# seervideodiffusion/SeerVideoLDM

Measured on AMD Instinct MI355X. Metric: UNet denoising steps/sec (12-frame 256^2 latent, 50-step DDIM), higher is better.
Workload: dtype bf16; 1 GPU; Sthv2 config: CFG batch 2 x 12 frames (2 cond + 10 predicted) x 32x32 latent, full-width SeerUNet 1.08G params, 50-step DDIM, scale 7.5; global_batch=1, parallelism=single, hip_graph=True

## Files before the change

### include/seer_hip.h

```cpp
#ifndef SEER_HIP_H
#define SEER_HIP_H

#include <stdint.h>

#ifdef __cplusplus
extern "C" {
#endif

#define SEER_OK 0
#define SEER_EINVAL (-22)
#define SEER_ENOSYS (-38)
#define SEER_ELAUNCH (-5)

#define SEER_DT_BF16 0
#define SEER_DT_F16 1

int seer_abi_version(void);
const char* seer_strerror(int code);
const char* seer_build_arch(void);

#define SEER_GEMM_PLAIN 0
#define SEER_GEMM_CONV3X3 1
#define SEER_EPI_GEGLU 1u
#define SEER_EPI_OUT_F32 2u
// ... 129 lines not shown

int64_t seer_groupnorm_workspace_floats(int32_t C, int32_t batch, int64_t rows_per_batch, int32_t groups);
int seer_groupnorm_stats(const void* x1, int32_t C1, const void* x2, int32_t C2, int32_t batch,
                         int64_t rows_per_batch, int32_t groups, float* stats, float* workspace, int32_t dtype, void* stream);
int seer_groupnorm_stats_from_colsums(const float* cs1, int32_t C1, int32_t phases1, int32_t tiles1, const float* cs2,
                                      int32_t C2, int32_t phases2, int32_t tiles2, int32_t batch, int32_t groups,
                                      float* stats, void* stream);
int seer_groupnorm_apply(const void* x1, int32_t C1, const void* x2, int32_t C2, int32_t batch,
                         int64_t rows_per_batch, int32_t groups, const float* stats, double count, float eps,
                         const float* gamma, const float* beta, int32_t silu, void* y, int32_t dtype, void* stream);
int seer_groupnorm_apply_from_colsums(const void* x1, int32_t C1, const void* x2, int32_t C2, const float* cs1, int32_t phases1,
                                      int32_t tiles1, const float* cs2, int32_t phases2, int32_t tiles2, int32_t batch,
                                      int64_t rows_per_batch, int32_t groups, double count, float eps, const float* gamma,
                                      const float* beta, int32_t silu, void* y, int32_t dtype, void* stream);
int seer_groupnorm_apply_fx(const void* x1, int32_t C1, const void* x2, int32_t C2, const int64_t* fx1, int32_t reps1,
                            const int64_t* fx2, int32_t reps2, int32_t batch, int64_t rows_per_batch, int32_t groups, double count, float eps, const float* gamma,
                            const float* beta, int32_t silu, void* y, float* stats_out, int32_t dtype, void* stream);
int seer_groupnorm_stats_fx(const void* x, int32_t C, int32_t batch, int64_t rows_per_batch, int64_t* fx, int32_t dtype,
                            void* stream);
int seer_ff_fused_c320(const void* a, int32_t lda, const void* wof, const float* bo, const void* h, int32_t ldh, const void* x,
                       int32_t ldx, void* y, int32_t ldy, int64_t M, const float* gamma, const float* beta, float eps,
                       const void* w1f, const float* b1, const void* wcf, const float* bcat, int64_t* colsum_fx, int64_t fx_rows,
                       int32_t fx_reps, float* colsum_tiles, int32_t dtype, void* stream);
typedef struct seer_rowchain_desc {
    const void* inp; int32_t ld_in;
    const float* gn_stats; const int64_t* gn_fx; int32_t gn_fx_reps;
    double gn_count; float gn_eps; const float* gn_gamma; const float* gn_beta; int64_t rows_per_batch; int32_t groups;
    const void* w1f; const float* b1; const void* res; int32_t ldr; void* h; int32_t ldh;
    const float* ln_gamma; const float* ln_beta; float ln_eps;
    const void* w2f; int32_t n2; void* out; int32_t ldo;
    float col_scale; int32_t scale_thirds;
    const float* rot_table; int32_t rot_tokens_per_batch, rot_pos_offset, rot_head_dim, rot_dim, rot_thirds;
    int64_t M;
    int32_t dtype;
} seer_rowchain_desc;
int seer_rowchain_c320(const seer_rowchain_desc* desc , void* stream);
int seer_rowchain_pack(const void* W, int32_t ld, int32_t n_mats, void* out, void* stream);
int seer_ff_fused_pack_w1(const void* w1, void* out, void* stream);
int seer_ff_fused_pack_wcat(const void* wcat, void* out, void* stream);
int seer_layernorm(const void* x, int64_t rows, int32_t C, int32_t ldx, const float* gamma, const float* beta,
                   float eps, void* y, int32_t ldy, int32_t dtype, void* stream);

int seer_softmax_rows(const void* x, int32_t x_is_f32, int64_t rows, int32_t n, int32_t ld, float scale, void* y,
                      int32_t ldy, int32_t dtype, void* stream);

int seer_timestep_embedding(const int64_t* t, int32_t B, int32_t dim, int32_t flip_sin_to_cos, float freq_shift,
                            float* out, void* stream);

int seer_linear_smallm(const float* x, int32_t B, int32_t K, const void* W, const float* bias, int32_t N,
                       int32_t silu_in, int32_t silu_out, float* y, int32_t dtype, void* stream);

int seer_conv_in(const float* x, int32_t B, int32_t Cin, int32_t F, int32_t H, int32_t W_, const float* Wt,
                 const float* bias, int32_t Cout, void* y, int32_t dtype, void* stream);
int seer_conv_out(const void* x, int32_t B, int32_t C0, int32_t F, int32_t H, int32_t W_, const float* Wt,
                  const float* bias, int32_t Cout, float* y, int32_t dtype, void* stream);

int seer_conv1x1_nchw_f32(const float* x, int32_t N, int32_t Cin, int32_t Cout, int32_t HW, const float* Wt,
                          const float* bias, float* y, void* stream);

int seer_cast_f32(const float* x, int64_t n, void* y, int32_t dtype, void* stream);
int seer_nchw_f32_to_nhwc_bf16(const float* x, int32_t N, int32_t C, int32_t HW, void* y, void* stream);
int seer_nhwc_bf16_to_nchw_f32(const void* x, int32_t N, int32_t C, int32_t HW, float* y, void* stream);

int seer_cfg_ddim_step(const float* eps, int32_t cfg, int32_t b, int32_t C, int32_t F_total, int32_t cond_f,
                       int32_t HW, float scale, const float* coef, int32_t index, const float* x,
                       const float* noise , float* x_prev, float* pred_x0, void* stream);

int seer_ddim_step_begin(const float* x0_emb , const float* x, int32_t b, int32_t reps, int32_t C,
                         int32_t f1, int32_t F_pred, int32_t HW, const int64_t* t_table, int32_t* step, float* sample,
                         int64_t* t_out, void* stream);
int seer_cfg_ddim_step_dev(const float* eps, int32_t cfg, int32_t b, int32_t C, int32_t F_total, int32_t cond_f, int32_t HW,
                           float scale, const float* coef, int32_t* step, const float* x, const float* noise, float* x_prev,
                           float* pred_x0, void* stream);

int seer_slot_step_begin(const float* x0_emb , const float* x, int32_t slots, int32_t reps, int32_t C,
                         int32_t f1, int32_t F_pred, int32_t HW, const int64_t* t_table, int32_t nsched, int32_t* step,
                         float* sample, int64_t* t_out, void* stream);
int seer_slot_cfg_ddim_step(const float* eps, int32_t slots, int32_t C, int32_t F_total, int32_t cond_f, int32_t HW,
                            const float* scale, const float* coef, int32_t nsched, int32_t* step, const float* x, float* x_prev,
                            float* pred_x0, void* stream);

int seer_cfg_ddim_invert_step(const float* eps, int32_t cfg, int32_t b, int32_t C, int32_t F_total, int32_t cond_f, int32_t HW,
                              float scale, const float* coef, int32_t index, const float* x, float* x_next,
                              float* pred_x0 , void* stream);
int seer_cfg_ddim_invert_step_dev(const float* eps, int32_t cfg, int32_t b, int32_t C, int32_t F_total, int32_t cond_f, int32_t HW,
                                  float scale, const float* coef, int32_t* step, const int32_t* limit, const float* x,
                                  float* x_next, float* pred_x0, void* stream);

int seer_philox_u32(uint64_t seed, uint64_t stream, uint32_t index, uint64_t first_block, int64_t n_blocks, uint32_t* out,
                    void* hip_stream);
int seer_philox_normal(uint64_t seed, uint32_t stream, uint32_t index, int64_t n, float* out, void* hip_stream);
int seer_cfg_ddim_step_rng(const float* eps, int32_t cfg, int32_t b, int32_t C, int32_t F_total, int32_t cond_f, int32_t HW,
                           float scale, const float* coef, int32_t index, const float* x, const uint32_t* seeds, float temperature,
                           float* x_prev, float* pred_x0, void* stream);
int seer_cfg_ddim_step_rng_dev(const float* eps, int32_t cfg, int32_t b, int32_t C, int32_t F_total, int32_t cond_f, int32_t HW,
                               float scale, const float* coef, int32_t* step, const float* x, const uint32_t* seeds,
                               float temperature, float* x_prev, float* pred_x0, void* stream);
int seer_slot_cfg_ddim_step_rng(const float* eps, int32_t slots, int32_t C, int32_t F_total, int32_t cond_f, int32_t HW,
                                const float* scale, const float* coef, int32_t nsched, int32_t* step, const float* x,
                                const uint32_t* seeds, const float* temperature, float* x_prev, float* pred_x0, void* stream);

int seer_q_sample(const float* x0, int32_t b, int64_t per_row, const float* coef, int32_t nsched, const int32_t* index,
                  const float* noise, const uint32_t* seeds, float* out, void* stream);
int seer_known_blend(float* x, const float* mask, const float* known, int32_t b, int32_t C, int32_t F_pred, int32_t HW,
                     const float* coef, int32_t index, const int32_t* step, const float* noise, const uint32_t* seeds, void* stream);
int seer_slot_known_blend(float* x, const float* mask, const float* known, int32_t slots, int32_t C, int32_t F_pred, int32_t HW,
// ... 110 lines not shown
```

### seervideoldm_amd/_lib.py

```python
from __future__ import annotations

import ctypes as C
import os
from pathlib import Path

_PKG = Path(__file__).resolve().parent
_LIB_PATH = _PKG / "lib" / "libseer_hip.so"
_lib = None

ABI_VERSION = 26

SEER_GEMM_PLAIN = 0
SEER_GEMM_CONV3X3 = 1
SEER_EPI_GEGLU = 1
SEER_EPI_OUT_F32 = 2
SEER_EPI_SILU = 4
SEER_EPI_TRANS_OUT = 8
SEER_EPI_ROTARY = 16
SEER_EPI_COLSCALE = 32
SEER_EPI_F16 = 64
SEER_EPI_QUICKGELU = 128
SEER_ENOSYS = -38
SEER_DT_BF16, SEER_DT_F16 = 0, 1
SEER_ATTN_Q_PRESCALED = 1
# ... 73 lines not shown


class AttnBwdDesc(C.Structure):
    _fields_ = [
        ("fwd", AttnDesc),
        ("dO", C.c_void_p), ("dQ", C.c_void_p), ("dK", C.c_void_p), ("dV", C.c_void_p),
        ("do_bs", C.c_int64), ("dq_bs", C.c_int64), ("dk_bs", C.c_int64), ("dv_bs", C.c_int64),
        ("do_ss", C.c_int32), ("dq_ss", C.c_int32), ("dk_ss", C.c_int32), ("dv_ss", C.c_int32),
        ("delta", C.c_void_p),
    ]


_vp, _i32, _i64, _f32, _f64 = C.c_void_p, C.c_int32, C.c_int64, C.c_float, C.c_double
_u32, _u64 = C.c_uint32, C.c_uint64

SIGNATURES = {
    "seer_abi_version": ([], C.c_int),
    "seer_strerror": ([C.c_int], C.c_char_p),
    "seer_build_arch": ([], C.c_char_p),
    "seer_gemm_bf16": ([C.POINTER(GemmDesc), _vp], C.c_int),
    "seer_gemm_workspace_bytes": ([C.POINTER(GemmDesc)], C.c_int64),
    "seer_gemm_colsum_rows": ([C.POINTER(GemmDesc)], C.c_int32),
    "seer_gemm_sync_bytes": ([C.POINTER(GemmDesc)], C.c_int64),
    "seer_gemm_rowstat_ok": ([C.POINTER(GemmDesc)], C.c_int32),
    "seer_gemm_lnfold_ok": ([C.POINTER(GemmDesc)], C.c_int32),
    "seer_gemm_plan": ([C.POINTER(GemmDesc), C.POINTER(C.c_int32)], C.c_int),
    "seer_attn_fwd": ([C.POINTER(AttnDesc), _vp], C.c_int),
    "seer_attn_causal64": ([_vp, _vp, _vp, _i32, _vp, _i32, _vp, _i32, _i32, _i32, _vp], C.c_int),
    "seer_embed_tokens": ([_vp, _i32, _i32, _vp, _i32, _vp, _i32, _i32, _vp, _i32, _vp], C.c_int),
    "seer_rotary_table": ([_vp, _i32, _i32, _vp, _vp], C.c_int),
    "seer_rotary_inplace": ([_vp, _i64, _i32, _i32, _i32, _i32, _i32, _i32, _i32, _i32, _vp, _vp], C.c_int),
    "seer_groupnorm_workspace_floats": ([_i32, _i32, _i64, _i32], C.c_int64),
    "seer_groupnorm_stats": ([_vp, _i32, _vp, _i32, _i32, _i64, _i32, _vp, _vp, _i32, _vp], C.c_int),
    "seer_groupnorm_stats_from_colsums": ([_vp, _i32, _i32, _i32, _vp, _i32, _i32, _i32, _i32, _i32, _vp, _vp], C.c_int),
    "seer_groupnorm_apply": ([_vp, _i32, _vp, _i32, _i32, _i64, _i32, _vp, _f64, _f32, _vp, _vp, _i32, _vp, _i32, _vp], C.c_int),
    "seer_groupnorm_apply_from_colsums": ([_vp, _i32, _vp, _i32, _vp, _i32, _i32, _vp, _i32, _i32, _i32, _i64, _i32, _f64, _f32, _vp, _vp, _i32,
                                           _vp, _i32, _vp], C.c_int),
    "seer_groupnorm_apply_fx": ([_vp, _i32, _vp, _i32, _vp, _i32, _vp, _i32, _i32, _i64, _i32, _f64, _f32, _vp, _vp, _i32, _vp, _vp, _i32, _vp],
                                 C.c_int),
    "seer_groupnorm_stats_fx": ([_vp, _i32, _i32, _i64, _vp, _i32, _vp], C.c_int),
    "seer_ff_fused_c320": ([_vp, _i32, _vp, _vp, _vp, _i32, _vp, _i32, _vp, _i32, _i64, _vp, _vp, C.c_float, _vp, _vp, _vp, _vp, _vp, _i64, _i32,
                            _vp, _i32, _vp], C.c_int),
    "seer_rowchain_c320": ([C.POINTER(RowChainDesc), _vp], C.c_int),
    "seer_rowchain_pack": ([_vp, _i32, _i32, _vp, _vp], C.c_int),
    "seer_ff_fused_pack_w1": ([_vp, _vp, _vp], C.c_int),
    "seer_ff_fused_pack_wcat": ([_vp, _vp, _vp], C.c_int),
    "seer_gemm_colsum_fx_layout": ([C.POINTER(GemmDesc), _i32, C.POINTER(C.c_int32)], C.c_int32),
    "seer_layernorm": ([_vp, _i64, _i32, _i32, _vp, _vp, _f32, _vp, _i32, _i32, _vp], C.c_int),
    "seer_softmax_rows": ([_vp, _i32, _i64, _i32, _i32, _f32, _vp, _i32, _i32, _vp], C.c_int),
    "seer_conv1x1_nchw_f32": ([_vp, _i32, _i32, _i32, _i32, _vp, _vp, _vp, _vp], C.c_int),
    "seer_timestep_embedding": ([_vp, _i32, _i32, _i32, _f32, _vp, _vp], C.c_int),
    "seer_linear_smallm": ([_vp, _i32, _i32, _vp, _vp, _i32, _i32, _i32, _vp, _i32, _vp], C.c_int),
    "seer_conv_in": ([_vp, _i32, _i32, _i32, _i32, _i32, _vp, _vp, _i32, _vp, _i32, _vp], C.c_int),
    "seer_conv_out": ([_vp, _i32, _i32, _i32, _i32, _i32, _vp, _vp, _i32, _vp, _i32, _vp], C.c_int),
    "seer_cast_f32": ([_vp, _i64, _vp, _i32, _vp], C.c_int),
    "seer_nchw_f32_to_nhwc_bf16": ([_vp, _i32, _i32, _i32, _vp, _vp], C.c_int),
    "seer_nhwc_bf16_to_nchw_f32": ([_vp, _i32, _i32, _i32, _vp, _vp], C.c_int),
    "seer_cfg_ddim_step": ([_vp, _i32, _i32, _i32, _i32, _i32, _i32, _f32, _vp, _i32, _vp, _vp, _vp, _vp, _vp], C.c_int),
    "seer_ddim_step_begin": ([_vp, _vp, _i32, _i32, _i32, _i32, _i32, _i32, _vp, _vp, _vp, _vp, _vp], C.c_int),
    "seer_cfg_ddim_step_dev": ([_vp, _i32, _i32, _i32, _i32, _i32, _i32, _f32, _vp, _vp, _vp, _vp, _vp, _vp, _vp], C.c_int),
    "seer_cfg_ddim_invert_step": ([_vp, _i32, _i32, _i32, _i32, _i32, _i32, _f32, _vp, _i32, _vp, _vp, _vp, _vp], C.c_int),
    "seer_cfg_ddim_invert_step_dev": ([_vp, _i32, _i32, _i32, _i32, _i32, _i32, _f32, _vp, _vp, _vp, _vp, _vp, _vp, _vp], C.c_int),
    "seer_slot_step_begin": ([_vp, _vp, _i32, _i32, _i32, _i32, _i32, _i32, _vp, _i32, _vp, _vp, _vp, _vp], C.c_int),
    "seer_slot_cfg_ddim_step": ([_vp, _i32, _i32, _i32, _i32, _i32, _vp, _vp, _i32, _vp, _vp, _vp, _vp, _vp], C.c_int),
    "seer_philox_u32": ([_u64, _u64, _u32, _u64, _i64, _vp, _vp], C.c_int),
    "seer_philox_normal": ([_u64, _u32, _u32, _i64, _vp, _vp], C.c_int),
    "seer_cfg_ddim_step_rng": ([_vp, _i32, _i32, _i32, _i32, _i32, _i32, _f32, _vp, _i32, _vp, _vp, _f32, _vp, _vp, _vp], C.c_int),
    "seer_cfg_ddim_step_rng_dev": ([_vp, _i32, _i32, _i32, _i32, _i32, _i32, _f32, _vp, _vp, _vp, _vp, _f32, _vp, _vp, _vp], C.c_int),
    "seer_slot_cfg_ddim_step_rng": ([_vp, _i32, _i32, _i32, _i32, _i32, _vp, _vp, _i32, _vp, _vp, _vp, _vp, _vp, _vp, _vp], C.c_int),
    "seer_q_sample": ([_vp, _i32, _i64, _vp, _i32, _vp, _vp, _vp, _vp, _vp], C.c_int),
    "seer_known_blend": ([_vp, _vp, _vp, _i32, _i32, _i32, _i32, _vp, _i32, _vp, _vp, _vp, _vp], C.c_int),
    "seer_slot_known_blend": ([_vp, _vp, _vp, _i32, _i32, _i32, _i32, _vp, _i32, _vp, _vp, _vp], C.c_int),
    "seer_slot_plms_step_begin": ([_vp, _vp, _vp, _i32, _i32, _i32, _i32, _i32, _i32, _vp, _i32, _vp, _vp, _vp, _vp, _vp], C.c_int),
    "seer_slot_cfg_plms_step": ([_vp, _i32, _i32, _i32, _i32, _i32, _vp, _vp, _i32, _vp, _vp, _vp, _vp, _vp, _vp, _vp, _vp],
                                C.c_int),
    "seer_cfg_plms_step": ([_vp, _i32, _i32, _i32, _i32, _i32, _i32, _f32, _vp, _i32, _i32, _vp, _vp, _vp, _vp, _vp, _vp, _vp,
                            _vp], C.c_int),
    "seer_cfg_plms_step_dev": ([_vp, _i32, _i32, _i32, _i32, _i32, _i32, _f32, _vp, _vp, _vp, _vp, _vp, _vp, _vp, _vp], C.c_int),
    "seer_clamp01": ([_vp, _i64, _vp], C.c_int),
    "seer_gaussian_sample": ([_vp, _i32, _i32, _i32, _vp, _vp, _vp], C.c_int),
    "seer_attn_bwd": ([C.POINTER(AttnBwdDesc), _vp], C.c_int),
    "seer_gemm_tn_workspace_bytes": ([_i32, _i32, _i32], C.c_int64),
    "seer_gemm_tn_f32": ([_vp, _i32, _vp, _i32, _i32, _i32, _i32, _vp, _vp, _vp, _i64, _vp], C.c_int),
    "seer_gemm_tn_grouped_workspace_bytes": ([C.POINTER(TnItem), _i32], C.c_int64),
    "seer_gemm_tn_grouped_f32": ([C.POINTER(TnItem), _i32, _vp, _i64, _vp], C.c_int),
    "seer_transpose_bf16": ([_vp, _i64, _i32, _i32, _vp, _i64, _vp], C.c_int),
    "seer_transpose_batched_bf16": ([_vp, _i32, _i64, _vp], C.c_int),
    "seer_colsum_workspace_floats": ([_i64, _i32], C.c_int64),
    "seer_colsum_bf16": ([_vp, _i64, _i32, _i32, _vp, _vp, _vp], C.c_int),
    "seer_layernorm_bwd": ([_vp, _vp, _i64, _i32, _i32, _i32, _vp, _f32, _vp, _i32, _vp, _i32, _vp, _vp, _vp, _vp], C.c_int),
    "seer_layernorm_bwd_slabs": ([_i64], C.c_int64),
    "seer_layernorm_bwd_partials": ([_vp, _vp, _i64, _i32, _i32, _i32, _vp, _f32, _vp, _i32, _vp, _i32, _vp, _vp], C.c_int),
    "seer_colfinal_grouped": ([C.POINTER(ColfinalItem), _i32, _vp], C.c_int),
    "seer_groupnorm_bwd_workspace_floats": ([_i32, _i32, _i64, _i32], C.c_int64),
    "seer_groupnorm_bwd": ([_vp, _i32, _vp, _i32, _i32, _i64, _i32, _vp, _f64, _f32, _vp, _vp, _i32, _vp, _vp, _vp, _vp, _vp,
                            _vp, _vp, _vp, _vp], C.c_int),
    "seer_geglu_fwd": ([_vp, _i64, _i32, _i32, _vp, _i32, _vp], C.c_int),
    "seer_geglu_bwd": ([_vp, _vp, _i64, _i32, _i32, _i32, _vp, _i32, _vp], C.c_int),
    "seer_add_bf16": ([_vp, _i32, _vp, _i32, _vp, _i32, _i64, _i32, _vp], C.c_int),
    "seer_sumpool2x_bf16": ([_vp, _i32, _i32, _i32, _i32, _vp, _vp], C.c_int),
    "seer_zero_insert2x_bf16": ([_vp, _i32, _i32, _i32, _i32, _vp, _vp], C.c_int),
    "seer_mse_loss_grad": ([_vp, _vp, _i32, _i32, _i32, _i32, _i32, _vp, _vp, _vp, _vp], C.c_int),
    "seer_text_loss_grad": ([_vp, _vp, _i32, _i32, _i64, _vp, _vp, _vp, _vp], C.c_int),
    "seer_conv_out_bwd": ([_vp, _i32, _i32, _i32, _i32, _i32, _vp, _i32, _vp, _vp], C.c_int),
    "seer_axpby_f32": ([_vp, _vp, _f32, _f32, _i64, _vp], C.c_int),
    "seer_sumsq_f32": ([_vp, _i64, _vp, _vp, _vp], C.c_int),
# ... 37 lines not shown
```

### seervideoldm_amd/csrc/elementwise.hip

```cpp
#include "seer_common.h"
#include <atomic>
#include <cstdint>

namespace {

__global__ void rotary_table_kernel(const float* __restrict__ freqs, int T, int half, float* __restrict__ cs) {
    const int i = blockIdx.x * blockDim.x + threadIdx.x;
    if (i >= T * half) return;
    const int pos = i / half, j = i - pos * half;
    const float ang = (float)pos * freqs[j];
    float s, c;
    sincosf(ang, &s, &c);
    cs[2 * i] = c;
    cs[2 * i + 1] = s;
}

__global__ void __launch_bounds__(256) rotary_kernel(bf16* __restrict__ x, int64_t rows, int ld, int col0_q, int col0_k,
                                                     int heads, int head_dim, int rot_dim, int tokens_per_batch,
                                                     int pos_offset, const float* __restrict__ cs) {
    const int64_t row = (int64_t)blockIdx.x * 4 + (threadIdx.x >> 6);
    if (row >= rows) return;
    const int lane = threadIdx.x & 63;
    const int cpr = rot_dim / 8;
    const int per_which = heads * cpr;
// ... 97 lines not shown
__global__ void __launch_bounds__(256) conv_in_kernel(const float* __restrict__ x, int B, int Cin, int F, int H, int Wd,
                                                      const float* __restrict__ Wt, const float* __restrict__ bias,
                                                      int Cout, bf16* __restrict__ y, int ppb) {
    extern __shared__ __attribute__((aligned(16))) float wsm[];
    const int nw = 9 * Cin * Cout;
    const int kk = 9 * Cin;
    float* patch = wsm + nw;
    for (int i = threadIdx.x * 4; i < nw; i += 1024) *reinterpret_cast<f32x4*>(wsm + i) = *reinterpret_cast<const f32x4*>(Wt + i);
    const int64_t npix = (int64_t)B * F * H * Wd;
    const int64_t p0 = (int64_t)blockIdx.x * ppb;
    const int np = (int)(p0 + ppb < npix ? ppb : npix - p0);
    const int64_t cstride = (int64_t)F * H * Wd;
    for (int i = threadIdx.x; i < np * kk; i += 256) {
        const int pp = i / kk, k = i - pp * kk;
        const int tap = k / Cin, ci = k - tap * Cin;
        const int64_t pix = p0 + pp;
        const int ox = (int)(pix % Wd);
        const int oy = (int)((pix / Wd) % H);
        const int f = (int)((pix / ((int64_t)Wd * H)) % F);
        const int b = (int)(pix / ((int64_t)Wd * H * F));
        const int iy = oy + tap / 3 - 1, ix = ox + tap % 3 - 1;
        float v = 0.f;
        if (iy >= 0 && iy < H && ix >= 0 && ix < Wd)
            v = x[(((int64_t)b * Cin + ci) * F + f) * H * Wd + (int64_t)iy * Wd + ix];
        patch[i] = v;
    }
    __syncthreads();
    const int cgroups = Cout / 8;
    const int npl = 256 / cgroups;
    const int pl = threadIdx.x / cgroups;
    const int cg = threadIdx.x - pl * cgroups;
    if (pl >= npl) return;
    float bv[8];
#pragma unroll
    for (int e = 0; e < 8; ++e) bv[e] = bias ? bias[cg * 8 + e] : 0.f;
    for (int pp = pl; pp < np; pp += npl) {
        float acc[8];
#pragma unroll
        for (int e = 0; e < 8; ++e) acc[e] = bv[e];
        const float* xp = patch + pp * kk;
        const float* wp = wsm + cg * 8;
#pragma unroll 4
        for (int k = 0; k < kk; ++k) {
            const float xv = xp[k];
            const f32x4 w0 = *reinterpret_cast<const f32x4*>(wp + k * Cout);
            const f32x4 w1 = *reinterpret_cast<const f32x4*>(wp + k * Cout + 4);
#pragma unroll
            for (int e = 0; e < 4; ++e) { acc[e] += xv * w0[e]; acc[4 + e] += xv * w1[e]; }
        }
        *reinterpret_cast<u32x4*>(y + (p0 + pp) * Cout + cg * 8) = pack8t<F16>(acc);
    }
}

template <int COUT, bool F16 = false>
__global__ void __launch_bounds__(256) conv_out_kernel(const bf16* __restrict__ x, int B, int C0, int F, int H, int Wd,
                                                       const float* __restrict__ Wt, const float* __restrict__ bias,
                                                       float* __restrict__ y, int ppb) {
    extern __shared__ __attribute__((aligned(16))) float wsm[];
    const int nw = COUT * 9 * C0;
    for (int i = threadIdx.x * 4; i < nw; i += 1024) *reinterpret_cast<f32x4*>(wsm + i) = *reinterpret_cast<const f32x4*>(Wt + i);
    __syncthreads();
    const int64_t npix = (int64_t)B * F * H * Wd;
    const int64_t p0 = (int64_t)blockIdx.x * ppb;
    const int64_t p1 = p0 + ppb < npix ? p0 + ppb : npix;
    const int lane = threadIdx.x & 63;
    const int nch = C0 / 8;
    for (int64_t pix = p0 + (threadIdx.x >> 6); pix < p1; pix += 4) {
        const int ox = (int)(pix % Wd);
        const int oy = (int)((pix / Wd) % H);
        const int64_t img = pix / ((int64_t)Wd * H);
        f32x2 acc[COUT];
#pragma unroll
        for (int o = 0; o < COUT; ++o) acc[o] = f32x2{0.f, 0.f};
        for (int item = lane; item < 9 * nch; item += 64) {
            const int tap = item / nch, ch = item - tap * nch;
            const int ky = tap / 3, kx = tap - 3 * ky;
            const int iy = oy + ky - 1, ix = ox + kx - 1;
            if (iy < 0 || iy >= H || ix < 0 || ix >= Wd) continue;
            const u32x4 v = *reinterpret_cast<const u32x4*>(x + ((img * H + iy) * Wd + ix) * C0 + ch * 8);
            float f[8];
            unpack8t<F16>(v, f);
#pragma unroll
            for (int o = 0; o < COUT; ++o) {
                const float* w = wsm + (o * 9 + tap) * C0 + ch * 8;
                const f32x4 w0 = *reinterpret_cast<const f32x4*>(w);
                const f32x4 w1 = *reinterpret_cast<const f32x4*>(w + 4);
                acc[o] = __builtin_elementwise_fma(f32x2{f[0], f[1]}, f32x2{w0[0], w0[1]}, acc[o]);
                acc[o] = __builtin_elementwise_fma(f32x2{f[2], f[3]}, f32x2{w0[2], w0[3]}, acc[o]);
                acc[o] = __builtin_elementwise_fma(f32x2{f[4], f[5]}, f32x2{w1[0], w1[1]}, acc[o]);
                acc[o] = __builtin_elementwise_fma(f32x2{f[6], f[7]}, f32x2{w1[2], w1[3]}, acc[o]);
            }
        }
        const int f_ = (int)(img % F);
        const int b = (int)(img / F);
#pragma unroll
        for (int o = 0; o < COUT; ++o) {
            const float v = wave_sum(acc[o][0] + acc[o][1]);
            if (lane == 0) y[((((int64_t)b * COUT + o) * F + f_) * H + oy) * Wd + ox] = v + (bias ? bias[o] : 0.f);
        }
    }
}

template <bool F16>
__global__ void cast_f32_bf16_kernel(const float* __restrict__ x, int64_t n, bf16* __restrict__ y) {
    const int64_t i = ((int64_t)blockIdx.x * blockDim.x + threadIdx.x) * 4;
    if (i + 3 < n) {
// ... 91 lines not shown
extern "C" int seer_rotary_inplace(void* x, int64_t rows, int32_t ld, int32_t col0_q, int32_t col0_k, int32_t heads,
                                   int32_t head_dim, int32_t rot_dim, int32_t tokens_per_batch, int32_t pos_offset,
                                   const float* cos_sin, void* stream) {
    if (!x || !cos_sin || rows <= 0 || heads <= 0 || rot_dim <= 0 || rot_dim % 8 || rot_dim > head_dim) return SEER_EINVAL;
    if (ld % 8 || col0_q % 8 || col0_k % 8 || head_dim % 8 || tokens_per_batch <= 0) return SEER_EINVAL;
    hipLaunchKernelGGL(rotary_kernel, dim3((unsigned)((rows + 3) / 4)), dim3(256), 0, S(stream),
                       reinterpret_cast<bf16*>(x), rows, ld, col0_q, col0_k, heads, head_dim, rot_dim, tokens_per_batch,
                       pos_offset, cos_sin);
    SEER_LAUNCH_CHECK();
    return SEER_OK;
}

extern "C" int seer_timestep_embedding(const int64_t* t, int32_t B, int32_t dim, int32_t flip_sin_to_cos,
                                       float freq_shift, float* out, void* stream) {
    if (!t || !out || B <= 0 || dim <= 0 || dim % 2) return SEER_EINVAL;
    const int n = B * dim / 2;
    hipLaunchKernelGGL(timestep_embedding_kernel, dim3((n + 255) / 256), dim3(256), 0, S(stream), t, B, dim,
                       flip_sin_to_cos, freq_shift, out);
    SEER_LAUNCH_CHECK();
    return SEER_OK;
}

template <typename K>
int ensure_lds(K kernel, size_t bytes, std::atomic<bool>* done) {
    if (bytes > 160 * 1024) return SEER_EINVAL;
    if (bytes > 64 * 1024 && !done->load(std::memory_order_acquire)) {
        if (hipFuncSetAttribute(reinterpret_cast<const void*>(kernel), hipFuncAttributeMaxDynamicSharedMemorySize, 160 * 1024) != hipSuccess)
            return SEER_ELAUNCH;
        done->store(true, std::memory_order_release);
    }
    return SEER_OK;
}

extern "C" int seer_linear_smallm(const float* x, int32_t B, int32_t K, const void* W, const float* bias, int32_t N,
                                  int32_t silu_in, int32_t silu_out, float* y, int32_t dtype, void* stream) {
    if (!x || !W || !y || B <= 0 || B > 8 || K <= 0 || K % 8 || N <= 0) return SEER_EINVAL;
    const size_t lds = (size_t)B * K * sizeof(float);
    static std::atomic<bool> done[4] = {{false}, {false}, {false}, {false}};
#define SEER_LSM(MB, R, GRID, FLAG)                                                                                                 \
    seer_dispatch_dtype(dtype, [&](auto f16) {                                                                                      \
        constexpr bool F16 = decltype(f16)::value;                                                                                  \
        const int rc = ensure_lds(linear_smallm_kernel<MB, R, F16>, lds, &done[FLAG + !F16]);                                       \
        if (rc != SEER_OK) return rc;                                                                                               \
        hipLaunchKernelGGL((linear_smallm_kernel<MB, R, F16>), dim3(GRID), dim3(256), lds, S(stream), x, B, K,                      \
                           reinterpret_cast<const bf16*>(W), bias, N, silu_in, silu_out, y);                                        \
        SEER_LAUNCH_CHECK();                                                                                                        \
        return SEER_OK;                                                                                                             \
    })
    if (B <= 2) return SEER_LSM(2, 4, (N + 15) / 16, 0);
    return SEER_LSM(8, 2, (N + 7) / 8, 2);
#undef SEER_LSM
}

extern "C" int seer_conv_in(const float* x, int32_t B, int32_t Cin, int32_t F, int32_t H, int32_t W_, const float* Wt,
                            const float* bias, int32_t Cout, void* y, int32_t dtype, void* stream) {
    static std::atomic<bool> done[2] = {{false}, {false}};
    return seer_dispatch_dtype(dtype, [&](auto f16) {
        constexpr bool F16 = decltype(f16)::value;
        if (!x || !Wt || !y || B <= 0 || Cin <= 0 || F <= 0 || H <= 0 || W_ <= 0 || Cout <= 0 || Cout % 8 || Cout > 2048)
            return SEER_EINVAL;
        const int ppb = 32;
        const size_t lds = ((size_t)9 * Cin * Cout + (size_t)ppb * 9 * Cin) * sizeof(float);
        const int rc = ensure_lds(conv_in_kernel<F16>, lds, &done[F16]);
        if (rc != SEER_OK) return rc;
        const int64_t npix = (int64_t)B * F * H * W_;
        hipLaunchKernelGGL(conv_in_kernel<F16>, dim3((unsigned)((npix + ppb - 1) / ppb)), dim3(256), lds, S(stream), x, B, Cin, F, H,
                           W_, Wt, bias, Cout, reinterpret_cast<bf16*>(y), ppb);
        SEER_LAUNCH_CHECK();
        return SEER_OK;
    });
}

extern "C" int seer_conv_out(const void* x, int32_t B, int32_t C0, int32_t F, int32_t H, int32_t W_, const float* Wt,
                             const float* bias, int32_t Cout, float* y, int32_t dtype, void* stream) {
    if (dtype != SEER_DT_BF16 && dtype != SEER_DT_F16) return SEER_EINVAL;
    if (!x || !Wt || !y || B <= 0 || C0 <= 0 || C0 % 8 || F <= 0 || H <= 0 || W_ <= 0) return SEER_EINVAL;
    const int64_t npix = (int64_t)B * F * H * W_;
    const int ppb = 32;
    dim3 grid((unsigned)((npix + ppb - 1) / ppb));
    const size_t lds = (size_t)Cout * 9 * C0 * sizeof(float);
    const bf16* xb = reinterpret_cast<const bf16*>(x);
    if (dtype == SEER_DT_F16) {
        if (Cout != 3) return SEER_ENOSYS;
        static std::atomic<bool> done16{false};
        const int rc = ensure_lds(conv_out_kernel<3, true>, lds, &done16);
        if (rc != SEER_OK) return rc;
        hipLaunchKernelGGL((conv_out_kernel<3, true>), grid, dim3(256), lds, S(stream), xb, B, C0, F, H, W_, Wt, bias, y, ppb);
    } else if (Cout == 4) {
        static std::atomic<bool> done{false};
        const int rc = ensure_lds(conv_out_kernel<4>, lds, &done);
        if (rc != SEER_OK) return rc;
        hipLaunchKernelGGL(conv_out_kernel<4>, grid, dim3(256), lds, S(stream), xb, B, C0, F, H, W_, Wt, bias, y, ppb);
    } else if (Cout == 3) {
        static std::atomic<bool> done{false};
        const int rc = ensure_lds(conv_out_kernel<3>, lds, &done);
        if (rc != SEER_OK) return rc;
        hipLaunchKernelGGL(conv_out_kernel<3>, grid, dim3(256), lds, S(stream), xb, B, C0, F, H, W_, Wt, bias, y, ppb);
    } else {
        return SEER_ENOSYS;
    }
    SEER_LAUNCH_CHECK();
    return SEER_OK;
}

extern "C" int seer_cast_f32(const float* x, int64_t n, void* y, int32_t dtype, void* stream) {
    return seer_dispatch_dtype(dtype, [&](auto f16) {
        if (!x || !y || n <= 0) return SEER_EINVAL;
        const int64_t nt = (n + 3) / 4;
        hipLaunchKernelGGL(cast_f32_bf16_kernel<decltype(f16)::value>, dim3((unsigned)((nt + 255) / 256)), dim3(256), 0, S(stream), x, n,
                           reinterpret_cast<bf16*>(y));
        SEER_LAUNCH_CHECK();
        return SEER_OK;
    });
}

extern "C" int seer_nchw_f32_to_nhwc_bf16(const float* x, int32_t N, int32_t C, int32_t HW, void* y, void* stream) {
    if (!x || !y || N <= 0 || C <= 0 || HW <= 0) return SEER_EINVAL;
    dim3 grid((HW + 31) / 32, (C + 31) / 32, N);
    hipLaunchKernelGGL(nchw_to_nhwc_kernel, grid, dim3(256), 0, S(stream), x, C, HW, reinterpret_cast<bf16*>(y));
    SEER_LAUNCH_CHECK();
    return SEER_OK;
}
extern "C" int seer_nhwc_bf16_to_nchw_f32(const void* x, int32_t N, int32_t C, int32_t HW, float* y, void* stream) {
// ... 46 lines not shown
```

### seervideoldm_amd/ops.py

```python
from __future__ import annotations

import ctypes as C
from typing import Optional

import torch

from . import _lib
from ._lib import AttnDesc, GemmDesc, check

bf16 = torch.bfloat16


def _stream() -> int:
    return torch.cuda.current_stream().cuda_stream


def _p(t: Optional[torch.Tensor]) -> Optional[int]:
    if t is None:
        return None
    if not t.is_cuda:
        raise _lib.SeerHipError("seervideoldm_amd kernels need tensors on a ROCm device (no CPU fallback)")
    return t.data_ptr()


# ... 682 lines not shown
    if h is not None:
        h.colsums = None
        h.rowstats = None
    return h, o


def softmax_rows(x: torch.Tensor, scale: float, out: Optional[torch.Tensor] = None, dtype=None) -> torch.Tensor:
    assert x.dtype in (bf16, f16, torch.float32) and x.is_cuda
    x2 = x.reshape(-1, x.shape[-1])
    assert x2.is_contiguous()
    if out is None:
        out = torch.empty(x.shape, device=x.device, dtype=dtype if dtype is not None else (x.dtype if x.dtype != torch.float32 else bf16))
    ldy = out.reshape(-1, out.shape[-1]).stride(0)
    dt = _req16(out, "out", None if x.dtype == torch.float32 else x)
    assert out.shape[-1] >= x2.shape[1] and out.numel() // out.shape[-1] == x2.shape[0]
    check(_lib.load().seer_softmax_rows(_p(x2), int(x.dtype == torch.float32), x2.shape[0], x2.shape[1], x2.stride(0),
                                        float(scale), _p(out), ldy, dt, _stream()), "seer_softmax_rows")
    return out


def conv1x1_nchw(x: torch.Tensor, w: torch.Tensor, bias: Optional[torch.Tensor]) -> torch.Tensor:
    _req(x, torch.float32, "x"); _req(w, torch.float32, "w")
    x = x.contiguous()
    N, Cin = x.shape[0], x.shape[1]
    HW = x.numel() // (N * Cin)
    Cout = w.shape[0]
    y = torch.empty((N, Cout) + tuple(x.shape[2:]), device=x.device, dtype=torch.float32)
    check(_lib.load().seer_conv1x1_nchw_f32(_p(x), N, Cin, Cout, HW, _p(w), _p(bias), _p(y), _stream()),
          "seer_conv1x1_nchw_f32")
    return y


def timestep_embedding(t: torch.Tensor, dim: int, flip_sin_to_cos: bool, freq_shift: float) -> torch.Tensor:
    _req(t, torch.int64, "timestep")
    out = torch.empty((t.numel(), dim), device=t.device, dtype=torch.float32)
    check(_lib.load().seer_timestep_embedding(_p(t), t.numel(), dim, int(flip_sin_to_cos), float(freq_shift), _p(out),
                                              _stream()), "seer_timestep_embedding")
    return out


def linear_smallm(x: torch.Tensor, w: torch.Tensor, bias: Optional[torch.Tensor], *, silu_in=False,
                  silu_out=False) -> torch.Tensor:
    _req(x, torch.float32, "x")
    dt = _req16(w, "w")
    assert x.is_contiguous() and w.is_contiguous()
    B, K = x.shape
    N = w.shape[0]
    y = torch.empty((B, N), device=x.device, dtype=torch.float32)
    check(_lib.load().seer_linear_smallm(_p(x), B, K, _p(w), _p(bias), N, int(silu_in), int(silu_out), _p(y), dt,
                                         _stream()), "seer_linear_smallm")
    return y


def conv_in(x: torch.Tensor, w_khwc: torch.Tensor, bias: torch.Tensor, dtype=bf16) -> torch.Tensor:
    _req(x, torch.float32, "x"); _req(w_khwc, torch.float32, "w")
    assert x.is_contiguous()
    B, Cin, F, H, W = x.shape
    Cout = w_khwc.shape[-1]
    y = torch.empty((B * F * H * W, Cout), device=x.device, dtype=dtype)
    dt = _req16(y, "y")
    check(_lib.load().seer_conv_in(_p(x), B, Cin, F, H, W, _p(w_khwc), _p(bias), Cout, _p(y), dt, _stream()),
          "seer_conv_in")
    return y


def conv_out(x: torch.Tensor, w_ohwc: torch.Tensor, bias: torch.Tensor, B: int, F: int, H: int, W: int, tile=0) -> torch.Tensor:
    dt = _req16(x, "x")
    Cout = w_ohwc.shape[0]
    y = torch.empty((B, Cout, F, H, W), device=x.device, dtype=torch.float32)
    if w_ohwc.dtype in (bf16, f16):
        _req16(w_ohwc, "w", x)
        C0 = x.shape[1]
        assert w_ohwc.dim() == 2 and w_ohwc.shape[1] == 9 * C0 and Cout % 4 == 0 and x.is_contiguous()
        M = F * H * W
        d = GemmDesc()
        d.A, d.W, d.C = _p(x), _p(w_ohwc), _p(y)
        d.M, d.N, d.K, d.K1 = M, Cout, 9 * C0, 9 * C0
        d.ldc = M
        _req(bias, torch.float32, "bias")
        d.bias = _p(bias)
        d.mode = _lib.SEER_GEMM_CONV3X3
        d.epilogue = _lib.SEER_EPI_TRANS_OUT | _lib.SEER_EPI_OUT_F32 | (_lib.SEER_EPI_F16 if dt else 0)
        d.Hin, d.Win, d.Cin, d.Hout, d.Wout, d.stride, d.upsample = H, W, C0, H, W, 1, 0
        d.batch, d.strideA, d.strideW, d.strideC = B, M * C0, 0, Cout * M
        d.tile = tile
        d.splits = 1
        _launch_gemm(d, x.device, "seer_gemm_bf16(conv_out)")
        return y
    _req(w_ohwc, torch.float32, "w")
    check(_lib.load().seer_conv_out(_p(x), B, x.shape[1], F, H, W, _p(w_ohwc), _p(bias), Cout, _p(y), dt, _stream()),
          "seer_conv_out")
    return y


def cast_bf16(x: torch.Tensor, dtype=bf16) -> torch.Tensor:
    _req(x, torch.float32, "x")
    x = x.contiguous()
    y = torch.empty(x.shape, device=x.device, dtype=dtype)
    check(_lib.load().seer_cast_f32(_p(x), x.numel(), _p(y), _req16(y, "y"), _stream()), "seer_cast_f32")
    return y


def nchw_to_nhwc_bf16(x: torch.Tensor) -> torch.Tensor:
    _req(x, torch.float32, "x")
    x = x.contiguous()
    N, Cc = x.shape[0], x.shape[1]
    HW = x.numel() // (N * Cc)
    y = torch.empty((N * HW, Cc), device=x.device, dtype=bf16)
    check(_lib.load().seer_nchw_f32_to_nhwc_bf16(_p(x), N, Cc, HW, _p(y), _stream()), "seer_nchw_f32_to_nhwc_bf16")
    return y


def nhwc_to_nchw_f32(x: torch.Tensor, N: int, H: int, W: int) -> torch.Tensor:
    _req(x, bf16, "x")
    Cc = x.shape[1]
# ... 345 lines not shown
```

### seervideoldm_amd/unet.py

```python
from __future__ import annotations

import json
import os
from collections import OrderedDict
from types import SimpleNamespace
from typing import Dict, List, Optional, Tuple, Union

import torch
import torch.nn as nn

from . import _lib
from . import ops as hip_ops
from . import synth
from .groupnorm import groupnorm, groupnorm_statistics
from .weights import geglu_row_order, pack_conv1x1, pack_conv3x3, pack_conv3x3_up_phases

bf16 = torch.bfloat16
MAX_WIN_SIZE, MAX_RATIO, MIN_WIN_SIZE = 8, 4, 4


class _Node(nn.Module):
    def forward(self, *a, **k):
        raise RuntimeError("container module: the forward pass lives in SeerUNet.forward")

# ... 583 lines not shown
            if H > MIN_WIN_SIZE:
                ws = MAX_WIN_SIZE if (H // MAX_WIN_SIZE) >= MAX_RATIO else MIN_WIN_SIZE
                ops.attention(qkv[:, :C], qkv[:, C:2 * C], qkv[:, 2 * C:], a, batch=B, heads=heads, head_dim=d,
                              Sq=Fr * ws * ws, Sk=Fr * ws * ws, causal=True, window=(ws, Fr, H, W), q_prescaled=True)
            else:
                ops.attention(qkv[:, :C], qkv[:, C:2 * C], qkv[:, 2 * C:], a, batch=B, heads=heads, head_dim=d,
                              Sq=Fr * HW, Sk=Fr * HW, causal=True, q_prescaled=True)
        skip_f = cond_frame if self.shard is None else self.shard.local_cond_frames(cond_frame)
        whole = skip_f <= 0 and not (self.inv and cond_frame > 0)
        if whole and self._ff_pre(p, tb, h):
            return self._ff_proj_out(p, tb, h, x, self._cb(B, Fr * HW), a=a)
        ops.gemm(a, w[tb + ".attn1.to_out.0.weight"], bias=w[tb + ".attn1.to_out.0.bias"], residual=h, out=h,
                 **({} if whole and self._ff_fused_rows(p, h) else self._rs()))
        if whole:
            return self._ff_proj_out(p, tb, h, x, self._cb(B, Fr * HW))
        elif skip_f < Fr:
            for b in range(B):
                self._ff(tb, h[b * Fr * HW + skip_f * HW:(b + 1) * Fr * HW])
        return ops.gemm(h, w[p + ".proj_out.weight"], bias=w[p + ".proj_out.bias"], residual=x,
                        colsum_batch=self._cb(B, Fr * HW))

    def n_groupnorms(self):
        return sum(1 for k in self.w if k.endswith(".weight") and
                   (k.endswith("norm1.weight") or k.endswith("norm2.weight") or k.endswith(".norm.weight") or
                    k == "conv_norm_out.weight") and "transformer_blocks" not in k)

    def _forward(self, sample, t, ctx_bf16, ctx_len, cond_frame, return_attn=False):
        ops, w = self.ops, self.w
        B, Cin, Fr, H, W = sample.shape
        boc, lpb, n = self.boc, self.lpb, len(self.boc)
        self._attn_list = [] if return_attn else None
        self._attn_wanted = {f"down_blocks.{i}.attentions.{lpb - 1}" for i in range(n - 1)} | {"mid_block.attentions.0"} | \
                            {f"up_blocks.{i}.attentions.{lpb}" for i in range(1, n)}
        self._ctx, self._ctx_len = ctx_bf16, ctx_len
        self._B = B
        self._stats_arena = torch.empty((self.n_groupnorms(), B, self.G, 2), device=sample.device, dtype=torch.float32)
        self._stats_i = 0
        self.gn_from_colsums = 0
        self.ln_folded = 0
        self.rowchains = 0
        self._fx = None
        small = (self._rows_all(Fr * H * W) if self.inv else B * Fr * H * W) <= FX_MAX_ROWS
        fx_gn = (self.gn_fx and self.gn_colsums) or self.inv
        self._ln_on = self.ln_fold and small
        if (fx_gn or self._ln_on) and hasattr(ops, "FxArena"):
            need = (self.n_groupnorms() + 16) * B * 4 * max(boc) * 2 + 5 * 16 * B * Fr * H * W * 2
            self._fx_arena = fx_arena(ops, sample, need, self._fx_arena, self._fx_retired)
            self._fx = self._fx_arena if fx_gn else None
        emb = ops.timestep_embedding(t, boc[0], self.cfg.flip_sin_to_cos, self.cfg.freq_shift)
        emb = ops.linear_smallm(emb, w["time_embedding.linear_1.weight"], w["time_embedding.linear_1.bias"], silu_out=True)
        emb = ops.linear_smallm(emb, w["time_embedding.linear_2.weight"], w["time_embedding.linear_2.bias"])
        self._temb = ops.linear_smallm(emb, w["temb_all.w"], w["temb_all.b"], silu_in=True)

        x = ops.conv_in(sample, w["conv_in.weight"], w["conv_in.bias"]) if self.dt == bf16 else \
            ops.conv_in(sample, w["conv_in.weight"], w["conv_in.bias"], dtype=self.dt)
        skips = [x]
        geo = (B, Fr, H, W)
        for i in range(n):
            p = f"down_blocks.{i}"
            for j in range(lpb):
                x = self._resnet(f"{p}.resnets.{j}", x, None, geo, feeds_transformer=i < n - 1)
                if i < n - 1:
                    x = self._text_transformer(f"{p}.attentions.{j}", x, geo)
                    x = self._temporal_transformer(f"{p}.temporal_attentions.{j}", x, geo, cond_frame)
                skips.append(x)
            if i < n - 1:
                x = ops.conv3x3(x, w[f"{p}.downsamplers.0.conv.weight"], B * Fr, geo[2], geo[3], stride=2,
                                bias=w[f"{p}.downsamplers.0.conv.bias"],
                                colsum_batch=self._cb(B, Fr * ((geo[2] - 1) // 2 + 1) * ((geo[3] - 1) // 2 + 1)))
                geo = (B, Fr, (geo[2] - 1) // 2 + 1, (geo[3] - 1) // 2 + 1)
                skips.append(x)
        x = self._resnet("mid_block.resnets.0", x, None, geo, feeds_transformer=True)
        x = self._text_transformer("mid_block.attentions.0", x, geo)
        x = self._temporal_transformer("mid_block.temporal_attentions.0", x, geo, cond_frame)
        x = self._resnet("mid_block.resnets.1", x, None, geo)
        for i in range(n):
            p = f"up_blocks.{i}"
            for j in range(lpb + 1):
                x = self._resnet(f"{p}.resnets.{j}", x, skips.pop(), geo, feeds_transformer=i > 0)
                if i > 0:
                    x = self._text_transformer(f"{p}.attentions.{j}", x, geo)
                    x = self._temporal_transformer(f"{p}.temporal_attentions.{j}", x, geo, cond_frame)
            if i < n - 1:
                x = ops.conv_up2x(x, w[f"{p}.upsamplers.0.conv.weight_up4"], B * Fr, geo[2], geo[3],
                                  bias=w[f"{p}.upsamplers.0.conv.bias"], colsum_batch=self._cb(B, Fr * 4 * geo[2] * geo[3]))
                geo = (B, Fr, geo[2] * 2, geo[3] * 2)
        x = self._gn(x, None, B, Fr * geo[2] * geo[3], "conv_norm_out", self.eps, True)
        out = ops.conv_out(x, w["conv_out.weight"], w["conv_out.bias"], B, Fr, geo[2], geo[3])
        if return_attn:
            attn, self._attn_list = self._attn_list, None
            return out, attn
        return out

    def _context(self, context: torch.Tensor):
        key = (context.data_ptr(), context._version, tuple(context.shape), context.dtype)
        if key != self._kv_key:
            c = context.reshape(-1, context.shape[-1])
            new = (self.ops.cast_bf16(c.float()) if self.dt == bf16 else self.ops.cast_bf16(c.float(), self.dt)) if c.dtype != self.dt else c
            old = getattr(self, "_ctx_bf16", None)
            if old is not None and old.shape == new.shape and self._kv_cache:
                old.copy_(new)
                for tb, kv in self._kv_cache.items():
                    self.ops.gemm(old, self.w[tb + ".attn2.kv"], out=kv)
            else:
                self._ctx_bf16 = new.contiguous().clone() if new.data_ptr() == c.data_ptr() else new
                self._kv_cache = {}
                self._graphs.clear()
            self._kv_key = key
# ... 109 lines not shown
```

Measured before the change: 101.6 steps/s.

## Add MFMA conv_in kernel with fused GroupNorm column-sum epilogue

Adds a new conv_in kernel for Cin=4 that computes the 3x3 input convolution with f32 MFMA instructions, keeping weights in registers instead of staging them in LDS. It can also emit per-block column sums and sums of squares of the bf16 output. The first resnet's GroupNorm can then skip a separate statistics pass over the activation. The UNet forward enables the colsum path when colsum batching applies and exact sharded statistics are not required. This adds a new reduction layout and register pressure in exchange for one fewer read of the conv_in output.

```diff
diff --git a/include/seer_hip.h b/include/seer_hip.h
--- a/include/seer_hip.h
+++ b/include/seer_hip.h
@@ -205,6 +205,10 @@
 
 int seer_conv_in(const float* x, int32_t B, int32_t Cin, int32_t F, int32_t H, int32_t W_, const float* Wt,
                  const float* bias, int32_t Cout, void* y, int32_t dtype, void* stream);
+int32_t seer_conv_in_colsum_rows(int64_t rows_per_batch, int32_t Cin, int32_t Cout);
+int seer_conv_in_colsums(const float* x, int32_t B, int32_t Cin, int32_t F, int32_t H, int32_t W_, const float* Wt,
+                         const float* bias, int32_t Cout, void* y, float* colsum, int32_t colsum_rows, int32_t dtype,
+                         void* stream);
 int seer_conv_out(const void* x, int32_t B, int32_t C0, int32_t F, int32_t H, int32_t W_, const float* Wt,
                   const float* bias, int32_t Cout, float* y, int32_t dtype, void* stream);
 
diff --git a/seervideoldm_amd/_lib.py b/seervideoldm_amd/_lib.py
--- a/seervideoldm_amd/_lib.py
+++ b/seervideoldm_amd/_lib.py
@@ -149,6 +149,8 @@
     "seer_timestep_embedding": ([_vp, _i32, _i32, _i32, _f32, _vp, _vp], C.c_int),
     "seer_linear_smallm": ([_vp, _i32, _i32, _vp, _vp, _i32, _i32, _i32, _vp, _i32, _vp], C.c_int),
     "seer_conv_in": ([_vp, _i32, _i32, _i32, _i32, _i32, _vp, _vp, _i32, _vp, _i32, _vp], C.c_int),
+    "seer_conv_in_colsum_rows": ([_i64, _i32, _i32], C.c_int32),
+    "seer_conv_in_colsums": ([_vp, _i32, _i32, _i32, _i32, _i32, _vp, _vp, _i32, _vp, _vp, _i32, _i32, _vp], C.c_int),
     "seer_conv_out": ([_vp, _i32, _i32, _i32, _i32, _i32, _vp, _vp, _i32, _vp, _i32, _vp], C.c_int),
     "seer_cast_f32": ([_vp, _i64, _vp, _i32, _vp], C.c_int),
     "seer_nchw_f32_to_nhwc_bf16": ([_vp, _i32, _i32, _i32, _vp, _vp], C.c_int),
diff --git a/seervideoldm_amd/csrc/elementwise.hip b/seervideoldm_amd/csrc/elementwise.hip
--- a/seervideoldm_amd/csrc/elementwise.hip
+++ b/seervideoldm_amd/csrc/elementwise.hip
@@ -173,6 +173,111 @@
     }
 }
 
+__device__ __forceinline__ float row16_sum(float v) {
+#define SEER_ROW_ROR(N) __builtin_bit_cast(float, __builtin_amdgcn_update_dpp(0, __builtin_bit_cast(int, v), 0x120 + (N), 0xf, 0xf, false))
+    v += SEER_ROW_ROR(8);
+    v += SEER_ROW_ROR(4);
+    v += SEER_ROW_ROR(2);
+    v += SEER_ROW_ROR(1);
+#undef SEER_ROW_ROR
+    return v;
+}
+
+template <bool F16, bool CS>
+__global__ void __launch_bounds__(512) conv_in4_kernel(const float* __restrict__ x, int B, int F, int H, int Wd,
+                                                       const float* __restrict__ Wt, const float* __restrict__ bias, int Cout,
+                                                       bf16* __restrict__ y, int ppb, float* __restrict__ cs) {
+    const int lane = threadIdx.x & 63, wave = __builtin_amdgcn_readfirstlane(threadIdx.x >> 6);
+    const int n = lane & 15, kb = lane >> 4;
+    const int cbase = wave * 64;
+    const int nmt = min(4, (Cout - cbase) / 16);
+    float w[4][9];
+    f32x4 bv[4];
+#pragma unroll
+    for (int mt = 0; mt < 4; ++mt) {
+        const int c = cbase + (mt < nmt ? mt : 0) * 16;
+#pragma unroll
+        for (int t = 0; t < 9; ++t) w[mt][t] = Wt[(t * 4 + kb) * Cout + c + n];
+        bv[mt] = bias ? *reinterpret_cast<const f32x4*>(bias + c + kb * 4) : f32x4{0.f, 0.f, 0.f, 0.f};
+    }
+    const int npix = B * F * H * Wd, plane = H * Wd;
+    const int p0 = blockIdx.x * ppb;
+    const int np = p0 + ppb < npix ? ppb : npix - p0;
+    float bx[2][9];
+    bool valid[2];
+    int pix[2];
+#pragma unroll
+    for (int s = 0; s < 2; ++s) {
+        valid[s] = s * 16 + n < np;
+        pix[s] = p0 + (valid[s] ? s * 16 + n : 0);
+        const int img = pix[s] / plane, r = pix[s] - img * plane;
+        const int oy = r / Wd, ox = r - oy * Wd, b = img / F;
+        const float* xb = x + ((int64_t)(b * 4 + kb) * F + (img - b * F)) * plane;
+#pragma unroll
+        for (int t = 0; t < 9; ++t) {
+            const int iy = oy + t / 3 - 1, ix = ox + t % 3 - 1;
+            const int iyc = min(max(iy, 0), H - 1), ixc = min(max(ix, 0), Wd - 1);
+            const float v = xb[iyc * Wd + ixc];
+            bx[s][t] = valid[s] && iy == iyc && ix == ixc ? v : 0.f;
+        }
+    }
+#pragma unroll
+    for (int mt = 0; mt < 4; ++mt) {
+#pragma unroll
+        for (int t = 0; t < 9; ++t) asm volatile("" ::"v"(w[mt][t]));
+        asm volatile("" ::"v"(bv[mt]));
+    }
+#pragma unroll
+    for (int s = 0; s < 2; ++s)
+#pragma unroll
+        for (int t = 0; t < 9; ++t) asm volatile("" ::"v"(bx[s][t]));
+    f32x4 sm[4], sq[4];
+#pragma unroll
+    for (int mt = 0; mt < 4; ++mt) sm[mt] = sq[mt] = f32x4{0.f, 0.f, 0.f, 0.f};
+#pragma unroll
+    for (int s = 0; s < 2; ++s) {
+        if (s * 16 >= np) break;
+        bf16* yp = y + (int64_t)pix[s] * Cout + cbase + kb * 4;
+#pragma unroll
+        for (int mt = 0; mt < 4; ++mt) {
+            if (mt < nmt) {
+                f32x4 acc = bv[mt];
+#pragma unroll
+                for (int t = 0; t < 9; ++t) acc = __builtin_amdgcn_mfma_f32_16x16x4f32(w[mt][t], bx[s][t], acc, 0, 0, 0);
+                const u32x2 o = {pack2t<F16>(acc[0], acc[1]), pack2t<F16>(acc[2], acc[3])};
+                if (valid[s]) *reinterpret_cast<u32x2*>(yp + mt * 16) = o;
+                if constexpr (CS) {
+                    const unsigned int keep = valid[s] ? 0xffffffffu : 0u;
+                    const f32x2 lo = unpack2t<F16>(o[0] & keep), hi = unpack2t<F16>(o[1] & keep);
+                    const f32x4 v = {lo[0], lo[1], hi[0], hi[1]};
+#pragma unroll
+                    for (int i = 0; i < 4; ++i) {
+                        sm[mt][i] = s == 0 ? v[i] : sm[mt][i] + v[i];
+                        sq[mt][i] = s == 0 ? v[i] * v[i] : __builtin_fmaf(v[i], v[i], sq[mt][i]);
+                    }
+                }
+            }
+        }
+    }
+    if constexpr (CS) {
+#pragma unroll
+        for (int mt = 0; mt < 4; ++mt) {
+            if (mt < nmt) {
+#pragma unroll
+                for (int i = 0; i < 4; ++i) {
+                    sm[mt][i] = row16_sum(sm[mt][i]);
+                    sq[mt][i] = row16_sum(sq[mt][i]);
+                }
+                if (n == 0) {
+                    float* o = cs + ((int64_t)blockIdx.x * Cout + cbase + mt * 16 + kb * 4) * 2;
+                    *reinterpret_cast<f32x4*>(o) = f32x4{sm[mt][0], sq[mt][0], sm[mt][1], sq[mt][1]};
+                    *reinterpret_cast<f32x4*>(o + 4) = f32x4{sm[mt][2], sq[mt][2], sm[mt][3], sq[mt][3]};
+                }
+            }
+        }
+    }
+}
+
 template <int COUT, bool F16 = false>
 __global__ void __launch_bounds__(256) conv_out_kernel(const bf16* __restrict__ x, int B, int C0, int F, int H, int Wd,
                                                        const float* __restrict__ Wt, const float* __restrict__ bias,
@@ -370,23 +475,53 @@
 #undef SEER_LSM
 }
 
-extern "C" int seer_conv_in(const float* x, int32_t B, int32_t Cin, int32_t F, int32_t H, int32_t W_, const float* Wt,
-                            const float* bias, int32_t Cout, void* y, int32_t dtype, void* stream) {
+static bool conv_in4_ok(int Cin, int Cout) { return Cin == 4 && Cout % 16 == 0 && Cout <= 512; }
+
+extern "C" int32_t seer_conv_in_colsum_rows(int64_t rows_per_batch, int32_t Cin, int32_t Cout) {
+    if (rows_per_batch <= 0 || Cout <= 0 || !conv_in4_ok(Cin, Cout)) return 0;
+    int d = 32;
+    while (rows_per_batch % d) --d;
+    return d;
+}
+
+extern "C" int seer_conv_in_colsums(const float* x, int32_t B, int32_t Cin, int32_t F, int32_t H, int32_t W_, const float* Wt,
+                                    const float* bias, int32_t Cout, void* y, float* colsum, int32_t colsum_rows, int32_t dtype,
+                                    void* stream) {
     static std::atomic<bool> done[2] = {{false}, {false}};
     return seer_dispatch_dtype(dtype, [&](auto f16) {
         constexpr bool F16 = decltype(f16)::value;
         if (!x || !Wt || !y || B <= 0 || Cin <= 0 || F <= 0 || H <= 0 || W_ <= 0 || Cout <= 0 || Cout % 8 || Cout > 2048)
             return SEER_EINVAL;
-        const int ppb = 32;
-        const size_t lds = ((size_t)9 * Cin * Cout + (size_t)ppb * 9 * Cin) * sizeof(float);
+        if (colsum && (colsum_rows <= 0 || colsum_rows > 32 || ((int64_t)F * H * W_) % colsum_rows)) return SEER_EINVAL;
+        const int ppb = colsum ? colsum_rows : 32;
+        const int64_t npix = (int64_t)B * F * H * W_;
+        const dim3 grid((unsigned)((npix + ppb - 1) / ppb));
+        const size_t lds = ((size_t)9 * Cin * Cout + (size_t)32 * 9 * Cin) * sizeof(float);
+        if (lds > 160 * 1024) return SEER_EINVAL;
+        if (npix < ((int64_t)1 << 31) - 64 && conv_in4_ok(Cin, Cout)) {
+            const dim3 block((unsigned)((Cout + 63) / 64 * 64));
+            if (colsum)
+                hipLaunchKernelGGL((conv_in4_kernel<F16, true>), grid, block, 0, S(stream), x, B, F, H, W_, Wt, bias, Cout,
+                                   reinterpret_cast<bf16*>(y), ppb, colsum);
+            else
+                hipLaunchKernelGGL((conv_in4_kernel<F16, false>), grid, block, 0, S(stream), x, B, F, H, W_, Wt, bias, Cout,
+                                   reinterpret_cast<bf16*>(y), ppb, (float*)nullptr);
+            SEER_LAUNCH_CHECK();
+            return SEER_OK;
+        }
+        if (colsum) return SEER_ENOSYS;
         const int rc = ensure_lds(conv_in_kernel<F16>, lds, &done[F16]);
         if (rc != SEER_OK) return rc;
-        const int64_t npix = (int64_t)B * F * H * W_;
-        hipLaunchKernelGGL(conv_in_kernel<F16>, dim3((unsigned)((npix + ppb - 1) / ppb)), dim3(256), lds, S(stream), x, B, Cin, F, H,
-                           W_, Wt, bias, Cout, reinterpret_cast<bf16*>(y), ppb);
+        hipLaunchKernelGGL(conv_in_kernel<F16>, grid, dim3(256), lds, S(stream), x, B, Cin, F, H, W_, Wt, bias, Cout,
+                           reinterpret_cast<bf16*>(y), ppb);
         SEER_LAUNCH_CHECK();
         return SEER_OK;
     });
+}
+
+extern "C" int seer_conv_in(const float* x, int32_t B, int32_t Cin, int32_t F, int32_t H, int32_t W_, const float* Wt,
+                            const float* bias, int32_t Cout, void* y, int32_t dtype, void* stream) {
+    return seer_conv_in_colsums(x, B, Cin, F, H, W_, Wt, bias, Cout, y, nullptr, 0, dtype, stream);
 }
 
 extern "C" int seer_conv_out(const void* x, int32_t B, int32_t C0, int32_t F, int32_t H, int32_t W_, const float* Wt,
diff --git a/seervideoldm_amd/ops.py b/seervideoldm_amd/ops.py
--- a/seervideoldm_amd/ops.py
+++ b/seervideoldm_amd/ops.py
@@ -758,15 +758,24 @@
     return y
 
 
-def conv_in(x: torch.Tensor, w_khwc: torch.Tensor, bias: torch.Tensor, dtype=bf16) -> torch.Tensor:
+CONV_IN_COLSUMS = True
+
+
+def conv_in(x: torch.Tensor, w_khwc: torch.Tensor, bias: torch.Tensor, dtype=bf16, colsum_batch=0) -> torch.Tensor:
     _req(x, torch.float32, "x"); _req(w_khwc, torch.float32, "w")
     assert x.is_contiguous()
     B, Cin, F, H, W = x.shape
     Cout = w_khwc.shape[-1]
     y = torch.empty((B * F * H * W, Cout), device=x.device, dtype=dtype)
     dt = _req16(y, "y")
-    check(_lib.load().seer_conv_in(_p(x), B, Cin, F, H, W, _p(w_khwc), _p(bias), Cout, _p(y), dt, _stream()),
-          "seer_conv_in")
+    lib = _lib.load()
+    rows = lib.seer_conv_in_colsum_rows(F * H * W, Cin, Cout) if colsum_batch == B else 0
+    cs = None
+    if rows > 0:
+        cs = ColSums(torch.empty((1, B * F * H * W // rows, Cout, 2), device=x.device, dtype=torch.float32), Cout, 1, B * F * H * W // rows)
+    check(lib.seer_conv_in_colsums(_p(x), B, Cin, F, H, W, _p(w_khwc), _p(bias), Cout, _p(y), _p(cs.buf) if cs else None, rows, dt,
+                                   _stream()), "seer_conv_in")
+    y.colsums = cs
     return y
 
 
diff --git a/seervideoldm_amd/unet.py b/seervideoldm_amd/unet.py
--- a/seervideoldm_amd/unet.py
+++ b/seervideoldm_amd/unet.py
@@ -659,8 +659,10 @@
         emb = ops.linear_smallm(emb, w["time_embedding.linear_2.weight"], w["time_embedding.linear_2.bias"])
         self._temb = ops.linear_smallm(emb, w["temb_all.w"], w["temb_all.b"], silu_in=True)
 
-        x = ops.conv_in(sample, w["conv_in.weight"], w["conv_in.bias"]) if self.dt == bf16 else \
-            ops.conv_in(sample, w["conv_in.weight"], w["conv_in.bias"], dtype=self.dt)
+        kw = {} if self.dt == bf16 else {"dtype": self.dt}
+        if self._cb(B, Fr * H * W) and not (self.shard is not None and self.shard.exact_stats) and getattr(ops, "CONV_IN_COLSUMS", False):
+            kw["colsum_batch"] = B
+        x = ops.conv_in(sample, w["conv_in.weight"], w["conv_in.bias"], **kw)
         skips = [x]
         geo = (B, Fr, H, W)
         for i in range(n):
```

After: 101.9 steps/s (median of 6 runs). Within noise of the previous version (+0.3%).
